# Ajax0564/VyomAI

Hardware: AMD Instinct MI355X
Metric: training tokens/sec (12L d=768 seq=512 GPT-style decoder, CLM) (higher is better)
Workload: dtype bf16; 1 GPU; configs[1]: GPT-style Decoder 12L d=768 h=12 RoPE vocab 50265, CLM training B=32/GPU seq=512, AdamW, bf16 kernels + fp32 masters; global_batch=32, seq_len=512, parallelism=dp1, attention=none, weights=deterministic recipe (vyomai_amd.recipe)

## Files before the change

include/vyom_hip.h:

```cpp
#ifndef VYOM_HIP_H
#define VYOM_HIP_H

#include <stdint.h>

#ifdef __cplusplus
extern "C" {
#endif

typedef enum { VY_F32 = 0, VY_BF16 = 1 } vy_dtype;

typedef enum {
  VY_OK = 0,
  VY_ERR_ARG = -1,
  VY_ERR_UNSUPPORTED = -2,
  VY_ERR_LAUNCH = -3
} vy_status;

typedef enum {
  VY_ACT_NONE = 0, VY_ACT_GELU_ERF = 1, VY_ACT_GELU_TANH = 2,
  VY_ACT_SILU = 3, VY_ACT_TANH = 4, VY_ACT_SIGMOID = 5, VY_ACT_RELU6 = 6, VY_ACT_LEAKY_RELU = 7
} vy_act;
#define VY_ACT_SAVE_DERIV 0x100

enum {
// ... 42 lines not shown
                        void* v_cache, int64_t max_blocks, int block_size, int64_t T, int h, int hk, int dh,
                        int dtype, void* stream);
int vy_paged_qknorm_rope_write(void* qkv, int64_t ld, const int32_t* positions, const int64_t* slot_mapping,
                               const float* cos_tab, const float* sin_tab, int64_t table_rows,
                               const float* q_scale, const float* k_scale, float eps, void* k_cache,
                               void* v_cache, int64_t max_blocks, int block_size, int64_t T, int h, int hk, int dh,
                               int dtype, void* stream);
int vy_attn_paged_decode(const void* q, int64_t q_ld, const int32_t* q_rows, const void* k_cache,
                         const void* v_cache, int64_t max_blocks, int block_size,
                         const int32_t* block_table, int64_t bt_stride, const int32_t* seqlens,
                         int64_t max_seqlen, void* out, int64_t o_ld, int64_t B, int h, int hk, int dh,
                         float scale, int n_split, void* ws, int64_t ws_bytes, int dtype, void* stream);
int64_t vy_attn_paged_decode_ws_bytes(int64_t B, int h, int hk, int dh, int64_t max_seqlen, int n_split, int dtype);
int vy_attn_paged_prefill(const void* q, int64_t q_ld, const void* k_cache, const void* v_cache,
                          int64_t max_blocks, int block_size, const int32_t* block_table, int64_t bt_stride,
                          const int32_t* cu_q, const int32_t* ctx_lens, int64_t n_seq, int64_t max_q,
                          int64_t max_kv, void* out, int64_t o_ld, int h, int hk, int dh, float scale,
                          int dtype, void* stream);
int vy_paged_gather(const void* k_cache, const void* v_cache, int64_t max_blocks, int block_size,
                    const int32_t* block_table, int64_t n_blocks, int64_t S, void* k_out, void* v_out,
                    int hk, int dh, int dtype, void* stream);

int vy_layernorm_fwd(const void* x, int64_t ldx, const void* gamma, const void* beta, void* y,
                     int64_t ldy, float* mean, float* rstd, int64_t M, int64_t N, float eps,
                     int dtype, void* stream);

int vy_rmsnorm_fwd(const void* x, int64_t ldx, const void* w, void* y, int64_t ldy, int64_t M,
                   int64_t N, float eps, float w_offset, int dtype, void* stream);

int vy_gated_act_fwd(const void* gate_up, int64_t ldg, void* out, int64_t ldo, int64_t M, int64_t I,
                     int act, int dtype, void* stream);

int vy_rmsnorm_bwd(const void* dy, int64_t lddy, const void* x, int64_t ldx, const void* w,
                   const void* add_to, int64_t ldadd, void* dx, int64_t lddx, float* dw, float beta,
                   float* ws, int64_t M, int64_t N, float eps, float w_offset, int dtype, void* stream);

int vy_gated_act_bwd(const void* d_act, int64_t lddo, const void* gate_up, int64_t ldg, void* d_gate_up,
                     int64_t lddg, int64_t M, int64_t I, int act, int dtype, void* stream);

int vy_rope_fwd(void* x, int64_t sb, int64_t sh, int64_t sl, const float* cos_tab,
                const float* sin_tab, int64_t pos0, int64_t B, int heads, int64_t L, int dh,
                int inverse, int dtype, void* stream);


int vy_linear_dgrad(const void* dy, int64_t lddy, const void* wt, int64_t ldwt, const void* pre,
                    int64_t ldpre, int act, const void* add_to, int64_t ldadd, const void* add_to2,
                    int64_t ldadd2, void* dx, int64_t lddx, int64_t M, int64_t N, int64_t K, int dtype,
                    void* stream);

int vy_linear_wgrad(const void* dy, int64_t lddy, const void* x, int64_t ldx, float* dw,
                    int64_t lddw, float* db, float beta, const float* alpha_dev, int64_t M, int64_t N,
                    int64_t K, int dtype, void* stream);

typedef struct vy_wgrad_desc {
  const void* dy; int64_t lddy;
  const void* x; int64_t ldx;
  float* dw; int64_t lddw;
  float* db;
  int64_t M, N, K;
} vy_wgrad_desc;
int vy_linear_wgrad_grouped(const vy_wgrad_desc* descs, int32_t n, int dtype, void* stream);

typedef struct vy_colsum_desc {
  float* ws; int32_t W, N;
  float* out0; float* out1;
  int32_t acc;
} vy_colsum_desc;
int vy_linear_wgrad_grouped_cs(const vy_wgrad_desc* descs, int32_t n, const vy_colsum_desc* cs, int32_t ncs, int dtype,
                               void* stream);

int64_t vy_layernorm_bwd_ws_rows(int64_t M);
int vy_layernorm_bwd(const void* dy, int64_t lddy, const void* x, int64_t ldx, const void* gamma,
                     const float* mean, const float* rstd, void* dx, int64_t lddx, float* dgamma,
                     float* dbeta, float beta, float* ws, int64_t M, int64_t N, int dtype,
                     void* stream);
int vy_layernorm_bwd_partial(const void* dy, int64_t lddy, const void* x, int64_t ldx, const void* gamma,
                             const float* mean, const float* rstd, void* dx, int64_t lddx, float* ws, int64_t M,
                             int64_t N, int dtype, void* stream);

int vy_attn_bwd(const void* q, int64_t q_sb, int64_t q_sh, int64_t q_sl,
                const void* k, int64_t k_sb, int64_t k_sh, int64_t k_sl,
                const void* v, int64_t v_sb, int64_t v_sh, int64_t v_sl,
                const void* out, const void* dout, int64_t o_sb, int64_t o_sl, const float* lse,
                float* delta_ws,
                void* dq, int64_t dq_sb, int64_t dq_sh, int64_t dq_sl,
                void* dk, int64_t dk_sb, int64_t dk_sh, int64_t dk_sl,
                void* dv, int64_t dv_sb, int64_t dv_sh, int64_t dv_sl,
                int mask_kind, int64_t start_pos, const uint8_t* keypad, int64_t kp_sb,
                const float* cos_tab, const float* sin_tab, int64_t rope_pos0,
                int64_t B, int h, int hk, int64_t L, int64_t S, int dh, float scale, int dtype,
                void* stream);

int vy_ddp_unique_id(void* id128);
int vy_ddp_init(const void* id128, int rank, int world);
int vy_ddp_world(void);
int vy_ddp_rank(void);
int vy_ddp_all_reduce_async(void* buf, int64_t count, int dtype, void* stream);
int vy_ddp_destroy(void);

int vy_adamw_step(float* p, const float* g, float* m, float* v, void* p_bf16, int64_t n, float lr,
                  float beta1, float beta2, float eps, float weight_decay, int64_t step,
                  float grad_scale, const float* grad_scale_dev, void* stream);
int vy_adamw_step_gated(float* p, const float* g, float* m, float* v, void* p_bf16, int64_t n, float lr,
                        float beta1, float beta2, float eps, float weight_decay, int64_t step,
                        float grad_scale, const float* grad_scale_dev, const float* gate, void* stream);

// ... 119 lines not shown
```

vyomai_amd/_lib.py:

```python
from __future__ import annotations

import ctypes as C
import os
from typing import Optional

_HERE = os.path.dirname(os.path.abspath(__file__))
LIB_PATH = os.environ.get("VY_LIB_PATH") or os.path.join(_HERE, "lib", "libvyom_hip.so")

VY_F32, VY_BF16 = 0, 1
ACT_NONE, ACT_GELU_ERF, ACT_GELU_TANH = 0, 1, 2
ACT_SILU, ACT_TANH, ACT_SIGMOID, ACT_RELU6, ACT_LEAKY_RELU = 3, 4, 5, 6, 7
ACT_SAVE_DERIV = 0x100
MASK_NONE, MASK_CAUSAL, MASK_KEYPAD, MASK_ADDITIVE = 0, 1, 2, 4

_p, _i64, _i, _f, _u64 = C.c_void_p, C.c_int64, C.c_int, C.c_float, C.c_uint64

PROTOTYPES = {
    "vy_linear_fwd": [_p, _i64, _p, _i64, _p, _p, _i64, _p, _i64, _p, _i64, _i64, _i64, _i, _i, _p],
    "vy_qkv_rope_fwd": [_p, _i64, _p, _i64, _p, _p, _p, _i64,
                        _p, _i64, _i64, _i64, _p, _i64, _i64, _i64, _p, _i64, _i64, _i64,
                        _i64, _i64, _i64, _i, _i, _i, _i, _p],
    "vy_attn_fwd": [_p, _i64, _i64, _i64, _p, _i64, _i64, _i64, _p, _i64, _i64, _i64,
                    _p, _i64, _i64, _p, _i, _i64, _p, _i64, _p, _i64, _i64,
                    _i64, _i, _i, _i64, _i64, _i, _f, _i, _p],
# ... 6 lines not shown
                             _p, _i64, _i, _p],
    "vy_attn_paged_prefill": [_p, _i64, _p, _p, _i64, _i, _p, _i64, _p, _p, _i64, _i64, _i64, _p, _i64, _i, _i, _i, _f,
                              _i, _p],
    "vy_paged_gather": [_p, _p, _i64, _i, _p, _i64, _i64, _p, _p, _i, _i, _i, _p],
    "vy_layernorm_fwd": [_p, _i64, _p, _p, _p, _i64, _p, _p, _i64, _i64, _f, _i, _p],
    "vy_rmsnorm_fwd": [_p, _i64, _p, _p, _i64, _i64, _i64, _f, _f, _i, _p],
    "vy_gated_act_fwd": [_p, _i64, _p, _i64, _i64, _i64, _i, _i, _p],
    "vy_rmsnorm_bwd": [_p, _i64, _p, _i64, _p, _p, _i64, _p, _i64, _p, _f, _p, _i64, _i64, _f, _f, _i, _p],
    "vy_gated_act_bwd": [_p, _i64, _p, _i64, _p, _i64, _i64, _i64, _i, _i, _p],
    "vy_rope_fwd": [_p, _i64, _i64, _i64, _p, _p, _i64, _i64, _i, _i64, _i, _i, _i, _p],
    "vy_linear_dgrad": [_p, _i64, _p, _i64, _p, _i64, _i, _p, _i64, _p, _i64, _p, _i64, _i64, _i64, _i64, _i, _p],
    "vy_linear_wgrad": [_p, _i64, _p, _i64, _p, _i64, _p, _f, _p, _i64, _i64, _i64, _i, _p],
    "vy_linear_wgrad_grouped": [_p, _i, _i, _p],
    "vy_linear_wgrad_grouped_cs": [_p, _i, _p, _i, _i, _p],
    "vy_layernorm_bwd_partial": [_p, _i64, _p, _i64, _p, _p, _p, _p, _i64, _p, _i64, _i64, _i, _p],
    "vy_layernorm_bwd": [_p, _i64, _p, _i64, _p, _p, _p, _p, _i64, _p, _p, _f, _p, _i64, _i64, _i, _p],
    "vy_attn_bwd": [_p, _i64, _i64, _i64, _p, _i64, _i64, _i64, _p, _i64, _i64, _i64,
                    _p, _p, _i64, _i64, _p, _p,
                    _p, _i64, _i64, _i64, _p, _i64, _i64, _i64, _p, _i64, _i64, _i64,
                    _i, _i64, _p, _i64, _p, _p, _i64, _i64, _i, _i, _i64, _i64, _i, _f, _i, _p],
    "vy_adamw_step": [_p, _p, _p, _p, _p, _i64, _f, _f, _f, _f, _f, _i64, _f, _p, _p],
    "vy_adamw_step_gated": [_p, _p, _p, _p, _p, _i64, _f, _f, _f, _f, _f, _i64, _f, _p, _p, _p],
    "vy_sumsq": [_p, _i64, _p, _p, _p],
    "vy_linear_dropout_fwd": [_p, _i64, _p, _i64, _p, _p, _i64, _p, _i64, _i64, _i64, _i64, _f, _u64, _u64, _i, _p],
    "vy_dropout": [_p, _i64, _p, _i64, _i64, _i64, _f, _u64, _u64, _i, _p],
    "vy_act_bwd": [_p, _i64, _p, _i64, _p, _i64, _i64, _i64, _i, _i, _p],
    "vy_xent_fwd": [_p, _i64, _p, _i64, _p, _p, _p, _i64, _i64, _p, _i, _p],
    "vy_xent_bwd": [_p, _i64, _p, _i64, _p, _p, _p, _i64, _i64, _i, _p],
    "vy_xent_fused": [_p, _i64, _p, _i64, _p, _p, _p, _p, _i64, _i64, _p, _i, _p],
    "vy_xent_sample_fwd": [_p, _i64, _p, _i64, _p, _p, _p, _p, _f, _u64, _u64, _i64, _i64, _p, _i, _p],
    "vy_xent_sample_fused": [_p, _i64, _p, _i64, _p, _p, _p, _p, _p, _f, _u64, _u64, _i64, _i64, _p, _i, _p],
    "vy_gumbel_noise": [_p, _i64, _i64, _i64, _u64, _u64, _p],
    "vy_bce_head_fwd": [_p, _i64, _p, _p, _p, _p, _p, _p, _i64, _i64, _i, _p],
    "vy_bce_head_bwd": [_p, _i64, _p, _p, _p, _p, _p, _p, _p, _i64, _p, _p, _i, _i64, _i64, _i, _p],
    "vy_mlm_mask": [_p, _i64, _p, _i, _f, _i64, _i64, _i64, _u64, _u64, _p, _p, _p, _p],
    "vy_logprob_fwd": [_p, _i64, _p, _p, _p, _p, _i64, _i64, _p, _i, _p],
    "vy_logprob_bwd": [_p, _i64, _p, _p, _p, _i64, _i64, _i, _p],
    "vy_logprob_fused": [_p, _i64, _p, _p, _p, _p, _i64, _i64, _p, _i, _p],
    "vy_transpose_batched": [_p, _i, _i, _i, _p],
    "vy_embedding_fwd": [_p, _i64, _p, _p, _i64, _i64, _i64, _i64, _p, _i, _p],
    "vy_embedding_bwd": [_p, _i64, _p, _p, _i64, _i64, _i64, _i64, _i64, _i, _p],
    "vy_transpose": [_p, _i64, _p, _i64, _i64, _i64, _i, _p],
    "vy_greedy_step": [_p, _i64, _i64, _i64, _i, _p, _i64, _i64, _p, _i64, _p, _i, _p, _p, _p],
    "vy_sampling_probs": [_p, _i64, _i64, _i64, _i, _f, _i, _f, _p, _i64, _p],
    "vy_decoder_step": [_p, _p, _i64, _p, _p, _p, _i64, _p],
    "vy_gemma_decoder_step": [_p, _p, _i64, _p, _i64, _p],
    "vy_cast": [_p, _p, _i64, _i, _i, _p],
    "vy_ddp_unique_id": [_p],
    "vy_ddp_init": [_p, _i, _i],
    "vy_ddp_all_reduce_async": [_p, _i64, _i, _p],
    "vy_ddp_destroy": [],
    "vy_set_concurrent_chains": [_i],
    "vy_workspace_set": [_p, _p, _i64],
}
OTHER_SYMBOLS = ["vy_last_error", "vy_abi_version", "vy_layernorm_bwd_ws_rows", "vy_decode_ws_bytes",
                 "vy_gemma_ws_bytes", "vy_ddp_world", "vy_ddp_rank", "vy_attn_paged_decode_ws_bytes"]
ALL_SYMBOLS = list(PROTOTYPES) + OTHER_SYMBOLS


class VyWgradDesc(C.Structure):
    _fields_ = [("dy", _p), ("lddy", _i64), ("x", _p), ("ldx", _i64), ("dw", _p), ("lddw", _i64), ("db", _p),
                ("M", _i64), ("N", _i64), ("K", _i64)]


class VyColsumDesc(C.Structure):
    _fields_ = [("ws", _p), ("W", C.c_int32), ("N", C.c_int32), ("out0", _p), ("out1", _p), ("acc", C.c_int32)]


class VyomHipError(RuntimeError):
    pass


_lib: Optional[C.CDLL] = None


def load() -> C.CDLL:
    global _lib
    if _lib is not None:
        return _lib
    if not os.path.exists(LIB_PATH):
        raise VyomHipError(
            f"{LIB_PATH} is missing: build it with `python -c 'import __graft_entry__ as g; g.build()'` "
            "(hipcc --offload-arch=gfx950).  vyomai_amd has no CPU or PyTorch fallback."
        )
    lib = C.CDLL(LIB_PATH)
    for name, argtypes in PROTOTYPES.items():
        fn = getattr(lib, name)
        fn.argtypes = argtypes
        fn.restype = C.c_int
    lib.vy_last_error.restype = C.c_char_p
    lib.vy_last_error.argtypes = []
    lib.vy_abi_version.restype = C.c_int
    lib.vy_layernorm_bwd_ws_rows.restype = C.c_int64
    lib.vy_layernorm_bwd_ws_rows.argtypes = [_i64]
    lib.vy_decode_ws_bytes.restype = C.c_int64
    lib.vy_decode_ws_bytes.argtypes = [C.c_int32] * 7
    lib.vy_attn_paged_decode_ws_bytes.restype = C.c_int64
    lib.vy_attn_paged_decode_ws_bytes.argtypes = [_i64, _i, _i, _i, _i64, _i, _i]
    _lib = lib
    return lib


def call(name: str, *args) -> None:
    lib = load()
    rc = getattr(lib, name)(*args)
    if rc != 0:
        raise VyomHipError(f"{name} failed ({rc}): {lib.vy_last_error().decode()}")


def dtype_code(torch_dtype) -> int:
    import torch

    if torch_dtype == torch.bfloat16:
        return VY_BF16
    if torch_dtype == torch.float32:
        return VY_F32
    raise VyomHipError(f"vyomai_amd kernels support float32 and bfloat16, got {torch_dtype}")
```

vyomai_amd/csrc/vy_bwd.hip:

```cpp
#include "vy_attn_tile.h"
#include <float.h>
#include <stdlib.h>
#include <string.h>

namespace {


__device__ __forceinline__ int xcd_remap(int bid, int nwg) {
  const int xcd = bid & 7, q = nwg >> 3, r = nwg & 7;
  return (xcd < r ? xcd * (q + 1) : r * (q + 1) + (xcd - r) * q) + (bid >> 3);
}

__device__ __forceinline__ bf16x8 tr_pair(const char* base, int row_bytes) {
  const s16x4 lo = __builtin_amdgcn_ds_read_tr16_b64_v4i16((VY_LDS s16x4*)(base));
  const s16x4 hi = __builtin_amdgcn_ds_read_tr16_b64_v4i16((VY_LDS s16x4*)(base + 8 * row_bytes));
  union { struct { s16x4 a, b; } s; bf16x8 v; } u;
  u.s.a = lo; u.s.b = hi;
  return u.v;
}

typedef __attribute__((ext_vector_type(2))) __bf16 bf16x2_t;

template <int BT, int MS_, bool MF16>
struct WgradTile {
// ... 17 lines not shown
    wave = wave_, m_begin = m_begin_, m_end = m_end_;
    nst = (m_end - m_begin + MS - 1) / MS;
    ragged = ((m_end - m_begin) % MS) != 0;
    zero = reinterpret_cast<const bf16*>(vy_zero16);
    sources(dY, lddy, n0, N, lane, a_ptr, a_step);
    sources(X, ldx, k0, K, lane, b_ptr, b_step);
  }
  __device__ __forceinline__ void sources(const bf16* __restrict__ src, int64_t ld, int c0, int C, int lane,
                                          const bf16* (&ptr)[PP], int64_t (&step)[PP]) {
#pragma unroll
    for (int t = 0; t < PP; ++t) {
      const int P = (wave * PP + t) * 1024 + lane * 16;
      const int r = P / ROWB, off = P % ROWB;
      const int col = (off ^ (((r & 3) << 6) | (MF16 ? ((r >> 2) & 1) << 5 : 0))) >> 1;
      const bool ok = c0 + col < C;
      row[t] = r;
      ptr[t] = ok ? src + (int64_t)(m_begin + r) * ld + c0 + col : zero;
      step[t] = ok ? (int64_t)MS * ld : 0;
    }
  }
  __device__ __forceinline__ void issue(const bf16* (&ptr)[PP], const int64_t (&step)[PP], int s, char* dst) {
    const bool tail = ragged && s == nst - 1;
    const int rows = m_end - (m_begin + s * MS);
#pragma unroll
    for (int t = 0; t < PP; ++t) {
      const bf16* p = (tail && row[t] >= rows) ? zero : ptr[t];
      __builtin_amdgcn_global_load_lds((const VY_GLOBAL void*)p, (VY_LDS void*)(dst + (wave * PP + t) * 1024), 16, 0, 0);
      ptr[t] += step[t];
    }
  }
  __device__ __forceinline__ void stage(int s, char* dst) {
    issue(a_ptr, a_step, s, dst);
    issue(b_ptr, b_step, s, dst + TILE);
  }
};

__device__ __forceinline__ float wgrad_db_dot(const bf16x8& a, float s) {
  const bf16x2_t ones2 = {(__bf16)1.0f, (__bf16)1.0f};
  union { bf16x8 v; bf16x2_t h[4]; } u_;
  u_.v = a;
#pragma unroll
  for (int e = 0; e < 4; ++e) s = __builtin_amdgcn_fdot2_f32_bf16(u_.h[e], ones2, s, false);
  return s;
}

template <class T>
struct WgradMma32 {
  static constexpr int TJ = T::WKT / 32, KS = T::MS / 16, ROWB = T::ROWB;
  f32x16 acc[2][TJ];
  float sdb[2];
  int fr, fh;
  unsigned a_lds[2], b_lds[TJ];

  __device__ __forceinline__ WgradMma32(const char* smem, int lane, int wn, int wk) {
#pragma unroll
    for (int i = 0; i < 2; ++i)
#pragma unroll
      for (int j = 0; j < TJ; ++j)
#pragma unroll
        for (int r = 0; r < 16; ++r) acc[i][j][r] = 0.f;
    sdb[0] = sdb[1] = 0.f;
    fr = lane & 31, fh = lane >> 5;
    const int li = lane & 15, g16 = (lane >> 4) & 1;
    const int tr_row = 4 * fh + (li >> 2);
    const int tr_sw = ((li >> 2) & 3) << 6;
    const int a_rd = (2 * (wn * 64 + 16 * g16 + 4 * (li & 3)));
    const int b_rd = (2 * (wk * T::WKT + 16 * g16 + 4 * (li & 3)));
#pragma unroll
    for (int i = 0; i < 2; ++i) a_lds[i] = vy_lds_addr(smem) + tr_row * ROWB + ((a_rd + 64 * i) ^ tr_sw);
#pragma unroll
    for (int j = 0; j < TJ; ++j) b_lds[j] = vy_lds_addr(smem) + tr_row * ROWB + ((b_rd + 64 * j) ^ tr_sw);
  }
  __device__ __forceinline__ void mma_stage(unsigned off, bool do_db) {
    unsigned a_base[2], b_base[TJ];
#pragma unroll
    for (int i = 0; i < 2; ++i) a_base[i] = a_lds[i] + off;
#pragma unroll
    for (int j = 0; j < TJ; ++j) b_base[j] = b_lds[j] + off;
    bf16x8 af[2][2], bfr[2][TJ];
    auto frags = [&](auto ks_c, bf16x8* a_, bf16x8* b_) {
      constexpr int ks = decltype(ks_c)::value;
#pragma unroll
      for (int i = 0; i < 2; ++i)
        a_[i] = vy_lds_tr16_pair_off<16 * ks * ROWB, (16 * ks + 8) * ROWB>(a_base[i]);
#pragma unroll
      for (int j = 0; j < TJ; ++j)
        b_[j] = vy_lds_tr16_pair_off<T::TILE + 16 * ks * ROWB, T::TILE + (16 * ks + 8) * ROWB>(b_base[j]);
    };
    frags(std::integral_constant<int, 0>{}, af[0], bfr[0]);
    vy_static_for<KS>([&](auto ks_c) {
      constexpr int ks = decltype(ks_c)::value;
      constexpr int c_ = ks & 1;
      if constexpr (ks < KS - 1) {
        frags(std::integral_constant<int, ks + 1>{}, af[c_ ^ 1], bfr[c_ ^ 1]);
        asm volatile("s_waitcnt lgkmcnt(%0)" ::"n"(2 * (2 + TJ)) : "memory");
      } else {
        asm volatile("s_waitcnt lgkmcnt(0)" ::: "memory");
      }
#pragma unroll
      for (int i = 0; i < 2; ++i) vy_tie(af[c_][i]);
#pragma unroll
      for (int j = 0; j < TJ; ++j) vy_tie(bfr[c_][j]);
#pragma unroll
      for (int i = 0; i < 2; ++i)
#pragma unroll
        for (int j = 0; j < TJ; ++j)
          acc[i][j] = __builtin_amdgcn_mfma_f32_32x32x16_bf16(af[c_][i], bfr[c_][j], acc[i][j], 0, 0, 0);
      if (do_db) {
#pragma unroll
        for (int i = 0; i < 2; ++i) sdb[i] = wgrad_db_dot(af[c_][i], sdb[i]);
      }
    });
  }
  __device__ __forceinline__ void epilogue(float* __restrict__ dW, int64_t lddw, float* __restrict__ db, bool do_db,
                                           float alpha, int nw, int kw, int N, int K) {
    if (do_db) {
#pragma unroll
      for (int i = 0; i < 2; ++i) {
        const float t_ = (sdb[i] + __shfl_xor(sdb[i], 32, 64)) * alpha;
        const int n = nw + 32 * i + fr;
        if (fh == 0 && n < N) atomicAdd(db + n, t_);
      }
    }
#pragma unroll
    for (int i = 0; i < 2; ++i)
#pragma unroll
      for (int j = 0; j < TJ; ++j) {
        const int k = kw + 32 * j + fr;
        if (k >= K) continue;
#pragma unroll
        for (int r = 0; r < 16; ++r) {
          const int n = nw + 32 * i + (r & 3) + 8 * (r >> 2) + 4 * fh;
          if (n < N) atomicAdd(dW + (int64_t)n * lddw + k, acc[i][j][r] * alpha);
        }
      }
  }
};

template <class T>
struct WgradMma16 {
  static constexpr int TI = 4, TJ = T::WKT / 16, KS = T::MS / 32, JH = TJ / 2, ROWB = T::ROWB;
  f32x4 acc[TI][TJ];
  float sdb[TI];
  int r16, kq;
  unsigned a_lds[TI], b_lds[TJ];

  __device__ __forceinline__ WgradMma16(const char* smem, int lane, int wn, int wk) {
#pragma unroll
    for (int i = 0; i < TI; ++i)
#pragma unroll
      for (int j = 0; j < TJ; ++j) acc[i][j] = f32x4{0.f, 0.f, 0.f, 0.f};
#pragma unroll
    for (int i = 0; i < TI; ++i) sdb[i] = 0.f;
    r16 = lane & 15, kq = lane >> 4;
    const int q_ = r16 >> 2, p_ = r16 & 3;
    const int sw16 = (q_ << 6) | ((kq & 1) << 5);
#pragma unroll
    for (int i = 0; i < TI; ++i) a_lds[i] = vy_lds_addr(smem) + (4 * kq + q_) * ROWB + ((2 * (wn * 64 + 16 * i + 4 * p_)) ^ sw16);
#pragma unroll
    for (int j = 0; j < TJ; ++j)
      b_lds[j] = vy_lds_addr(smem) + (4 * kq + q_) * ROWB + ((2 * (wk * T::WKT + 16 * j + 4 * p_)) ^ sw16);
  }
  __device__ __forceinline__ void mma_stage(unsigned off, bool do_db) {
    unsigned a_base[TI], b_base[TJ];
#pragma unroll
    for (int i = 0; i < TI; ++i) a_base[i] = a_lds[i] + off;
#pragma unroll
    for (int j = 0; j < TJ; ++j) b_base[j] = b_lds[j] + off;
    vy_static_for<KS>([&](auto ks_c) {
      constexpr int ks = decltype(ks_c)::value;
      bf16x8 af[TI], bfr[TJ];
      vy_static_for<TI>([&](auto i_c) {
        constexpr int i = decltype(i_c)::value;
        af[i] = vy_lds_tr16_pair_off<32 * ks * ROWB, (32 * ks + 16) * ROWB>(a_base[i]);
      });
      vy_static_for<TJ>([&](auto j_c) {
        constexpr int j = decltype(j_c)::value;
        bfr[j] = vy_lds_tr16_pair_off<T::TILE + 32 * ks * ROWB, T::TILE + (32 * ks + 16) * ROWB>(b_base[j]);
      });
      asm volatile("s_waitcnt lgkmcnt(%0)" ::"n"(2 * JH) : "memory");
#pragma unroll
      for (int i = 0; i < TI; ++i) vy_tie(af[i]);
#pragma unroll
      for (int j = 0; j < JH; ++j) vy_tie(bfr[j]);
#pragma unroll
      for (int i = 0; i < TI; ++i)
#pragma unroll
        for (int j = 0; j < JH; ++j)
          acc[i][j] = __builtin_amdgcn_mfma_f32_16x16x32_bf16(af[i], bfr[j], acc[i][j], 0, 0, 0);
      asm volatile("s_waitcnt lgkmcnt(0)" ::: "memory");
#pragma unroll
      for (int j = JH; j < TJ; ++j) vy_tie(bfr[j]);
#pragma unroll
      for (int i = 0; i < TI; ++i)
#pragma unroll
        for (int j = JH; j < TJ; ++j)
          acc[i][j] = __builtin_amdgcn_mfma_f32_16x16x32_bf16(af[i], bfr[j], acc[i][j], 0, 0, 0);
      if (do_db) {
#pragma unroll
        for (int i = 0; i < TI; ++i) sdb[i] = wgrad_db_dot(af[i], sdb[i]);
      }
    });
  }
  __device__ __forceinline__ void epilogue(float* __restrict__ dW, int64_t lddw, float* __restrict__ db, bool do_db,
                                           float alpha, int nw, int kw, int N, int K) {
    if (do_db) {
#pragma unroll
      for (int i = 0; i < TI; ++i) {
        float t_ = sdb[i];
        t_ += __shfl_xor(t_, 16, 64);
        t_ += __shfl_xor(t_, 32, 64);
        const int n = nw + 16 * i + r16;
        if (kq == 0 && n < N) atomicAdd(db + n, t_ * alpha);
      }
    }
    const bool hi = kq >= 2;
#pragma unroll
    for (int i = 0; i < TI; ++i)
#pragma unroll
      for (int jp = 0; jp < JH; ++jp) {
        const int k = kw + 16 * (2 * jp + (hi ? 1 : 0)) + r16;
#pragma unroll
        for (int r = 0; r < 4; ++r) {
          const unsigned x = __builtin_bit_cast(unsigned, acc[i][2 * jp][r] * alpha);
          const unsigned y = __builtin_bit_cast(unsigned, acc[i][2 * jp + 1][r] * alpha);
          auto sw = __builtin_amdgcn_permlane32_swap(x, y, false, false);
          const int nlo = nw + 16 * i + 4 * (kq & 1) + r;
          if (k < K) {
            if (nlo < N) atomicAdd(dW + (int64_t)nlo * lddw + k, __builtin_bit_cast(float, (unsigned)sw[0]));
            if (nlo + 8 < N) atomicAdd(dW + (int64_t)(nlo + 8) * lddw + k, __builtin_bit_cast(float, (unsigned)sw[1]));
          }
        }
      }
  }
};

template <int BN, int BKW, int MS, int NS, bool MF16>
__device__ __forceinline__ void wgrad_tn_bf16_body(
    const bf16* __restrict__ dY, int64_t lddy, const bf16* __restrict__ X, int64_t ldx,
    float* __restrict__ dW, int64_t lddw, float* __restrict__ db, const float* __restrict__ alpha_dev,
    int M, int N, int K, int tiles_k, int tiles_nk, int m_chunk, int diag, int wg) {
  static_assert(BN == BKW && ((BN == 128 && MS == 64 && NS == 2) || (BN == 256 && MS == 32 && NS == 4)),
                "built shapes: 128 x 128 x 64 in 2 stages, 256 x 256 x 32 in 4");
  typedef WgradTile<BN, MS, MF16> Tile;
  typedef std::conditional_t<MF16, WgradMma16<Tile>, WgradMma32<Tile>> Mma;
  constexpr int STAGE = Tile::STAGE, PS = 2 * Tile::PP;
  __shared__ __attribute__((aligned(16))) char smem[NS * STAGE];
  const int tid = threadIdx.x, lane = tid & 63;
  const int wave = __builtin_amdgcn_readfirstlane(tid >> 6);
  const int wn = wave >> 1, wk = wave & 1;
  const int split = wg / tiles_nk, t2 = wg - split * tiles_nk;
  const int tile_n = t2 / tiles_k, tile_k = t2 - tile_n * tiles_k;
  const int n0 = tile_n * BN, k0 = tile_k * BKW;
  const int m_begin = split * m_chunk;
  const int m_end = min(M, m_begin + m_chunk);
  if (m_begin >= m_end) return;

  Tile t(dY, lddy, X, ldx, n0, k0, N, K, m_begin, m_end, wave, lane);
  const bool do_db = db != nullptr && tile_k == 0 && wk == 0;
  Mma mma(smem, lane, wn, wk);
  const int nst = t.nst;
#pragma unroll
  for (int s_ = 0; s_ < NS - 1; ++s_)
    if (s_ < nst) t.stage(s_, smem + s_ * STAGE);
  for (int s = 0; s < nst; ++s) {
    const int younger = min(NS - 2, nst - 1 - s);
    if (younger >= 2) asm volatile("s_waitcnt vmcnt(%0)" ::"n"(2 * PS) : "memory");
    else if (younger == 1) asm volatile("s_waitcnt vmcnt(%0)" ::"n"(PS) : "memory");
    else asm volatile("s_waitcnt vmcnt(0)" ::: "memory");
    __builtin_amdgcn_s_barrier();
    asm volatile("" ::: "memory");
    if (s + NS - 1 < nst) t.stage(s + NS - 1, smem + (s + NS - 1) % NS * STAGE);
    mma.mma_stage(s % NS * STAGE, do_db);
  }
  if (diag == 1) {
    if (mma.acc[0][0][0] == 12345.678f) dW[0] = 1.f;
    return;
  }
  const float alpha = alpha_dev ? *alpha_dev : 1.0f;
  mma.epilogue(dW, lddw, db, do_db, alpha, n0 + wn * 64, k0 + wk * Tile::WKT, N, K);
}

template <int BN, int BKW, int MS, int NS, bool MF16>
__global__ __launch_bounds__(BN * 2, BN == 128 ? 2 : 1) void wgrad_tn_bf16_kernel(
    const bf16* __restrict__ dY, int64_t lddy, const bf16* __restrict__ X, int64_t ldx,
    float* __restrict__ dW, int64_t lddw, float* __restrict__ db, const float* __restrict__ alpha_dev,
    int M, int N, int K, int tiles_k, int tiles_nk, int m_chunk, int diag) {
  wgrad_tn_bf16_body<BN, BKW, MS, NS, MF16>(dY, lddy, X, ldx, dW, lddw, db, alpha_dev, M, N, K, tiles_k, tiles_nk, m_chunk,
                                            diag, xcd_remap(blockIdx.x, gridDim.x));
}

struct WgradItem {
  const bf16* dY; const bf16* X; float* dW; float* db;
  int64_t lddy, ldx, lddw;
  int M, N, K, tiles_k, tiles_nk, m_chunk, item0;
};
struct WgradGroup { WgradItem g[8]; int n; };

struct ColsumItem { const float* ws; float* out0; float* out1; int W, N, rps, acc, blk0; };
struct ColsumGroup { ColsumItem c[8]; int n; int items; };

__device__ __forceinline__ void colsum_slab_block(const ColsumItem& it, int blk) {
  __shared__ float red[2][2][4][64];
  const int tid = threadIdx.x;
  const int c = tid & 63, g = (tid >> 6) & 3, h = tid >> 8;
  const int n = blk * 64 + c;
  const int W = it.W, N = it.N, rps = it.rps;
  const float* __restrict__ ws = it.ws;
  const bool one = rps >= W;
  float ta = 0.f, tb = 0.f;
  for (int s0 = 0; s0 * rps < W; s0 += 2) {
    const int w0 = (s0 + h) * rps, w1 = min(W, w0 + rps);
    float a = 0.f, b = 0.f;
    if (n < N) {
      for (int wb = w0 + g; wb < w1; wb += 32) {
        float av[8], bv[8];
#pragma unroll
        for (int i = 0; i < 8; ++i) {
          const int w = wb + 4 * i;
          const int wc = w < w1 ? w : wb;
          av[i] = ws[(int64_t)wc * N + n];
          bv[i] = ws[(int64_t)(W + wc) * N + n];
        }
#pragma unroll
        for (int i = 0; i < 8; ++i)
          if (wb + 4 * i < w1) { a += av[i]; b += bv[i]; }
      }
    }
    red[h][0][g][c] = a; red[h][1][g][c] = b;
    __syncthreads();
    if (tid < 64) {
#pragma unroll
      for (int hh = 0; hh < 2; ++hh)
        if ((s0 + hh) * rps < W) {
          const float sa = red[hh][0][0][c] + red[hh][0][1][c] + red[hh][0][2][c] + red[hh][0][3][c];
          const float sb = red[hh][1][0][c] + red[hh][1][1][c] + red[hh][1][2][c] + red[hh][1][3][c];
          ta = one ? sa : ta + sa;
          tb = one ? sb : tb + sb;
        }
    }
    __syncthreads();
  }
// ... 388 lines not shown
    const int n = n0 + 4 * ty + i;
    if (n >= N) continue;
#pragma unroll
    for (int j = 0; j < 4; ++j) {
      const int k = k0 + 4 * tx + j;
      if (k < K) atomicAdd(dW + (int64_t)n * lddw + k, alpha * acc[i][j]);
    }
  }
  if (db && k0 == 0) {
    sb[lr][lc] = colsum;
    __syncthreads();
    if (tid < 64 && n0 + tid < N) atomicAdd(db + n0 + tid, alpha * (sb[0][tid] + sb[1][tid] + sb[2][tid] + sb[3][tid]));
  }
}

int wgrad_f32(const char* who, const void* dy, int64_t lddy, const void* x, int64_t ldx, float* dw, int64_t lddw, float* db,
              float beta, const float* alpha_dev, int64_t M, int64_t N, int64_t K, hipStream_t st) {
  if (beta == 0.f) {
    if (hipMemset2DAsync(dw, lddw * sizeof(float), 0, K * sizeof(float), N, st) != hipSuccess)
      VY_FAIL(VY_ERR_LAUNCH, "%s: memset failed", who);
    if (db && hipMemsetAsync(db, 0, N * sizeof(float), st) != hipSuccess) VY_FAIL(VY_ERR_LAUNCH, "%s: memset failed", who);
  }
  const int tiles_k = (int)vy_cdiv(K, 64), tiles = (int)vy_cdiv(N, 64) * tiles_k;
  int64_t splits = vy_cdiv(1024, tiles);
  const int64_t max_splits = vy_cdiv(M, 64);
  if (splits > max_splits) splits = max_splits;
  if (splits < 1) splits = 1;
  const int64_t m_chunk = vy_cdiv(vy_cdiv(M, splits), 16) * 16;
  splits = vy_cdiv(M, m_chunk);
  hipLaunchKernelGGL(wgrad_tn_f32_kernel, dim3((unsigned)(tiles * splits)), dim3(256), 0, st, (const float*)dy, lddy,
                     (const float*)x, ldx, dw, lddw, db, alpha_dev, (int)M, (int)N, (int)K, tiles_k, tiles, (int)m_chunk);
  VY_CHECK_LAUNCH(who);
  return VY_OK;
}

bool wgrad_bf16_operands_ok(const void* dy, int64_t lddy, const void* x, int64_t ldx, int64_t N, int64_t K) {
  return !(K % 8 || lddy % 8 || ldx % 8 || lddy < vy_cdiv(N, 8) * 8 || (uintptr_t)dy % 16 || (uintptr_t)x % 16);
}

struct WgradSplit { int64_t splits, m_chunk; };
WgradSplit wgrad_split(int64_t M, int64_t want) {
  const int64_t max_splits = vy_cdiv(M, 256);
  if (want > max_splits) want = max_splits;
  if (want < 1) want = 1;
  const int64_t m_chunk = vy_cdiv(vy_cdiv(M, want), 64) * 64;
  return {vy_cdiv(M, m_chunk), m_chunk};
}

int wgrad_env(const char* name, int dflt) { const char* e = getenv(name); return e ? atoi(e) : dflt; }

int wgrad_m16() { static const int v = wgrad_env("VY_WGRAD_M16", 1); return v; }
int wgrad_diag() { static const int v = wgrad_env("VY_WGRAD_DIAG", 0); return v; }

}

extern "C" int vy_linear_wgrad(const void* dy, int64_t lddy, const void* x, int64_t ldx, float* dw,
                               int64_t lddw, float* db, float beta, const float* alpha_dev, int64_t M,
                               int64_t N, int64_t K, int dtype, void* stream) {
  const char* who = "vy_linear_wgrad";
  if (dtype != VY_BF16 && dtype != VY_F32) VY_FAIL(VY_ERR_ARG, "%s: bad dtype %d", who, dtype);
  if (!dy || !x || !dw || M <= 0 || N <= 0 || K <= 0) VY_FAIL(VY_ERR_ARG, "%s: bad arguments", who);
  if (dtype == VY_F32) {
    if (beta != 0.f && beta != 1.f) VY_FAIL(VY_ERR_ARG, "%s: beta must be 0 or 1", who);
    return wgrad_f32(who, dy, lddy, x, ldx, dw, lddw, db, beta, alpha_dev, M, N, K, (hipStream_t)stream);
  }
  if (!wgrad_bf16_operands_ok(dy, lddy, x, ldx, N, K))
    VY_FAIL(VY_ERR_ARG, "%s: K and leading dimensions must be multiples of 8 (lddy >= roundup8(N)), operands 16-byte aligned", who);
  if (beta != 0.f && beta != 1.f) VY_FAIL(VY_ERR_ARG, "%s: beta must be 0 or 1", who);
  static const int wv = wgrad_env("VY_WGRAD_VARIANT", -1);
  static const int tgt = wgrad_env("VY_WGRAD_TARGET", 0);
  if (wv != -1 && wv != 0 && wv != 8)
    VY_FAIL(VY_ERR_UNSUPPORTED, "%s: VY_WGRAD_VARIANT=%d was removed (the values left are 0 and 8; unset selects by shape)", who, wv);
  hipStream_t st = (hipStream_t)stream;
  if (beta == 0.f) {
    if (hipMemset2DAsync(dw, lddw * sizeof(float), 0, K * sizeof(float), N, st) != hipSuccess)
      VY_FAIL(VY_ERR_LAUNCH, "%s: memset failed", who);
    if (db && hipMemsetAsync(db, 0, N * sizeof(float), st) != hipSuccess)
      VY_FAIL(VY_ERR_LAUNCH, "%s: memset failed", who);
  }
  const bool big = wv < 0 ? (N >= 8192 && M >= 4096) : wv == 8;
  const int BT = big ? 256 : 128;
  const int tiles_k = (int)vy_cdiv(K, BT), tiles = (int)vy_cdiv(N, BT) * tiles_k;
  const WgradSplit sp = wgrad_split(M, tgt > 0 ? vy_cdiv(tgt, tiles) : big ? 256 / tiles : vy_cdiv(384, tiles));
  const int w16 = wgrad_m16();
  auto kernel = big ? (w16 ? wgrad_tn_bf16_kernel<256, 256, 32, 4, true> : wgrad_tn_bf16_kernel<256, 256, 32, 4, false>)
                    : (w16 >= 2 ? wgrad_tn_bf16_kernel<128, 128, 64, 2, true> : wgrad_tn_bf16_kernel<128, 128, 64, 2, false>);
  hipLaunchKernelGGL(kernel, dim3((unsigned)(tiles * sp.splits)), dim3(BT * 2), 0, st, (const bf16*)dy, lddy, (const bf16*)x,
                     ldx, dw, lddw, db, alpha_dev, (int)M, (int)N, (int)K, tiles_k, tiles, (int)sp.m_chunk, wgrad_diag());
  VY_CHECK_LAUNCH(who);
  return VY_OK;
}

static int wgrad_grouped(const char* who, const vy_wgrad_desc* descs, int32_t n, const vy_colsum_desc* cs, int32_t ncs,
                        int dtype, void* stream) {
  if (dtype != VY_BF16 && dtype != VY_F32) VY_FAIL(VY_ERR_ARG, "%s: bad dtype %d", who, dtype);
  if (n < 0 || n > 8 || (n > 0 && !descs) || ncs < 0 || ncs > 8 || (ncs > 0 && !cs) || n + ncs == 0)
    VY_FAIL(VY_ERR_ARG, "%s: 1..8 descriptors", who);
  for (int i = 0; i < ncs; ++i)
    if (!cs[i].ws || cs[i].W <= 0 || cs[i].N <= 0 || (cs[i].acc != 0 && cs[i].acc != 1))
      VY_FAIL(VY_ERR_ARG, "%s: column-sum descriptor %d: bad arguments", who, i);
  if (dtype == VY_F32) {
    for (int i = 0; i < ncs; ++i)
      if (int rc = vy_ln_colsum(cs[i].ws, cs[i].W, cs[i].N, cs[i].out0, cs[i].out1, cs[i].acc, (hipStream_t)stream)) return rc;
    for (int i = 0; i < n; ++i) {
      const vy_wgrad_desc& d = descs[i];
      if (!d.dy || !d.x || !d.dw || d.M <= 0 || d.N <= 0 || d.K <= 0) VY_FAIL(VY_ERR_ARG, "%s: descriptor %d: bad arguments", who, i);
      if (int rc = wgrad_f32(who, d.dy, d.lddy, d.x, d.ldx, d.dw, d.lddw, d.db, 1.f, nullptr, d.M, d.N, d.K, (hipStream_t)stream)) return rc;
    }
    return VY_OK;
  }
  int64_t tiles_total = 0;
  for (int i = 0; i < n; ++i) {
    const vy_wgrad_desc& d = descs[i];
    if (!d.dy || !d.x || !d.dw || d.M <= 0 || d.N <= 0 || d.K <= 0) VY_FAIL(VY_ERR_ARG, "%s: descriptor %d: bad arguments", who, i);
    if (!wgrad_bf16_operands_ok(d.dy, d.lddy, d.x, d.ldx, d.N, d.K))
      VY_FAIL(VY_ERR_ARG, "%s: descriptor %d: K and leading dimensions must be multiples of 8, operands 16-byte aligned", who, i);
    tiles_total += vy_cdiv(d.N, 256) * vy_cdiv(d.K, 256);
  }
  static const int tgt = wgrad_env("VY_WGRAD_GROUP_TARGET", 256);
  WgradGroup grp;
  memset(&grp, 0, sizeof(grp));
  grp.n = n;
  int64_t items = 0;
  for (int i = 0; i < n; ++i) {
    const vy_wgrad_desc& d = descs[i];
    const int64_t tiles_k = vy_cdiv(d.K, 256), tiles = vy_cdiv(d.N, 256) * tiles_k;
    const WgradSplit sp = wgrad_split(d.M, tgt / tiles_total);
    WgradItem& it = grp.g[i];
    it.dY = (const bf16*)d.dy; it.X = (const bf16*)d.x; it.dW = d.dw; it.db = d.db;
    it.lddy = d.lddy; it.ldx = d.ldx; it.lddw = d.lddw;
    it.M = (int)d.M; it.N = (int)d.N; it.K = (int)d.K;
    it.tiles_k = (int)tiles_k; it.tiles_nk = (int)tiles; it.m_chunk = (int)sp.m_chunk; it.item0 = (int)items;
    items += tiles * sp.splits;
  }
  for (int i = n; i < 8; ++i) grp.g[i] = grp.g[0];
  ColsumGroup cg;
  memset(&cg, 0, sizeof(cg));
// ... 554 lines not shown
```

Measured before the change: 872,800 tokens/s.

## Add persistent load-balanced ranged wgrad kernel for large-N weight gradients

Adds a persistent wgrad kernel for the 256x256 tile path, launched with one workgroup per CU. Each workgroup walks a contiguous range of (N-tile, M-block) segments for a fixed K-tile and runs the staged MMA ring on each segment. It writes each segment's partial result through the existing epilogue, then zeroes its accumulators and continues. This targets the tail imbalance of the old fixed grid of tiles×splits blocks on large-vocabulary shapes such as the LM head. The cost is more epilogue writes when one workgroup spans several N-tiles or splits a tile, plus new debug hooks for overriding and inspecting the plan.

Result: no change. 881,500 tokens/s (median of 6 runs) (+1.0%).

```diff
diff --git a/include/vyom_hip.h b/include/vyom_hip.h
--- a/include/vyom_hip.h
+++ b/include/vyom_hip.h
@@ -118,6 +118,9 @@
                     int64_t lddw, float* db, float beta, const float* alpha_dev, int64_t M, int64_t N,
                     int64_t K, int dtype, void* stream);
 
+int vy_debug_set_wgrad_balance(int on, int slots);
+int vy_debug_wgrad_plan(int64_t M, int64_t N, int64_t K, int slots, int target, int wg, int32_t* out, int cap);
+
 typedef struct vy_wgrad_desc {
   const void* dy; int64_t lddy;
   const void* x; int64_t ldx;
diff --git a/vyomai_amd/_lib.py b/vyomai_amd/_lib.py
--- a/vyomai_amd/_lib.py
+++ b/vyomai_amd/_lib.py
@@ -82,9 +82,11 @@
     "vy_ddp_destroy": [],
     "vy_set_concurrent_chains": [_i],
     "vy_workspace_set": [_p, _p, _i64],
+    "vy_debug_set_wgrad_balance": [_i, _i],
 }
 OTHER_SYMBOLS = ["vy_last_error", "vy_abi_version", "vy_layernorm_bwd_ws_rows", "vy_decode_ws_bytes",
-                 "vy_gemma_ws_bytes", "vy_ddp_world", "vy_ddp_rank", "vy_attn_paged_decode_ws_bytes"]
+                 "vy_gemma_ws_bytes", "vy_ddp_world", "vy_ddp_rank", "vy_attn_paged_decode_ws_bytes",
+                 "vy_debug_wgrad_plan"]
 ALL_SYMBOLS = list(PROTOTYPES) + OTHER_SYMBOLS
 
 
@@ -127,6 +129,8 @@
     lib.vy_decode_ws_bytes.argtypes = [C.c_int32] * 7
     lib.vy_attn_paged_decode_ws_bytes.restype = C.c_int64
     lib.vy_attn_paged_decode_ws_bytes.argtypes = [_i64, _i, _i, _i, _i64, _i, _i]
+    lib.vy_debug_wgrad_plan.restype = C.c_int
+    lib.vy_debug_wgrad_plan.argtypes = [_i64, _i64, _i64, _i, _i, _i, C.POINTER(C.c_int32), _i]
     _lib = lib
     return lib
 
diff --git a/vyomai_amd/csrc/vy_bwd.hip b/vyomai_amd/csrc/vy_bwd.hip
--- a/vyomai_amd/csrc/vy_bwd.hip
+++ b/vyomai_amd/csrc/vy_bwd.hip
@@ -93,7 +93,7 @@
   int fr, fh;
   unsigned a_lds[2], b_lds[TJ];
 
-  __device__ __forceinline__ WgradMma32(const char* smem, int lane, int wn, int wk) {
+  __device__ __forceinline__ void zero() {
 #pragma unroll
     for (int i = 0; i < 2; ++i)
 #pragma unroll
@@ -101,6 +101,9 @@
 #pragma unroll
         for (int r = 0; r < 16; ++r) acc[i][j][r] = 0.f;
     sdb[0] = sdb[1] = 0.f;
+  }
+  __device__ __forceinline__ WgradMma32(const char* smem, int lane, int wn, int wk) {
+    zero();
     fr = lane & 31, fh = lane >> 5;
     const int li = lane & 15, g16 = (lane >> 4) & 1;
     const int tr_row = 4 * fh + (li >> 2);
@@ -186,13 +189,16 @@
   int r16, kq;
   unsigned a_lds[TI], b_lds[TJ];
 
+  __device__ __forceinline__ void zero() {
+#pragma unroll
+    for (int i = 0; i < TI; ++i)
+#pragma unroll
+      for (int j = 0; j < TJ; ++j) acc[i][j] = f32x4{0.f, 0.f, 0.f, 0.f};
+#pragma unroll
+    for (int i = 0; i < TI; ++i) sdb[i] = 0.f;
+  }
   __device__ __forceinline__ WgradMma16(const char* smem, int lane, int wn, int wk) {
-#pragma unroll
-    for (int i = 0; i < TI; ++i)
-#pragma unroll
-      for (int j = 0; j < TJ; ++j) acc[i][j] = f32x4{0.f, 0.f, 0.f, 0.f};
-#pragma unroll
-    for (int i = 0; i < TI; ++i) sdb[i] = 0.f;
+    zero();
     r16 = lane & 15, kq = lane >> 4;
     const int q_ = r16 >> 2, p_ = r16 & 3;
     const int sw16 = (q_ << 6) | ((kq & 1) << 5);
@@ -276,30 +282,9 @@
   }
 };
 
-template <int BN, int BKW, int MS, int NS, bool MF16>
-__device__ __forceinline__ void wgrad_tn_bf16_body(
-    const bf16* __restrict__ dY, int64_t lddy, const bf16* __restrict__ X, int64_t ldx,
-    float* __restrict__ dW, int64_t lddw, float* __restrict__ db, const float* __restrict__ alpha_dev,
-    int M, int N, int K, int tiles_k, int tiles_nk, int m_chunk, int diag, int wg) {
-  static_assert(BN == BKW && ((BN == 128 && MS == 64 && NS == 2) || (BN == 256 && MS == 32 && NS == 4)),
-                "built shapes: 128 x 128 x 64 in 2 stages, 256 x 256 x 32 in 4");
-  typedef WgradTile<BN, MS, MF16> Tile;
-  typedef std::conditional_t<MF16, WgradMma16<Tile>, WgradMma32<Tile>> Mma;
+template <int NS, class Tile, class Mma>
+__device__ __forceinline__ void wgrad_ring(Tile& t, Mma& mma, char* smem, bool do_db) {
   constexpr int STAGE = Tile::STAGE, PS = 2 * Tile::PP;
-  __shared__ __attribute__((aligned(16))) char smem[NS * STAGE];
-  const int tid = threadIdx.x, lane = tid & 63;
-  const int wave = __builtin_amdgcn_readfirstlane(tid >> 6);
-  const int wn = wave >> 1, wk = wave & 1;
-  const int split = wg / tiles_nk, t2 = wg - split * tiles_nk;
-  const int tile_n = t2 / tiles_k, tile_k = t2 - tile_n * tiles_k;
-  const int n0 = tile_n * BN, k0 = tile_k * BKW;
-  const int m_begin = split * m_chunk;
-  const int m_end = min(M, m_begin + m_chunk);
-  if (m_begin >= m_end) return;
-
-  Tile t(dY, lddy, X, ldx, n0, k0, N, K, m_begin, m_end, wave, lane);
-  const bool do_db = db != nullptr && tile_k == 0 && wk == 0;
-  Mma mma(smem, lane, wn, wk);
   const int nst = t.nst;
 #pragma unroll
   for (int s_ = 0; s_ < NS - 1; ++s_)
@@ -314,6 +299,32 @@
     if (s + NS - 1 < nst) t.stage(s + NS - 1, smem + (s + NS - 1) % NS * STAGE);
     mma.mma_stage(s % NS * STAGE, do_db);
   }
+}
+
+template <int BN, int BKW, int MS, int NS, bool MF16>
+__device__ __forceinline__ void wgrad_tn_bf16_body(
+    const bf16* __restrict__ dY, int64_t lddy, const bf16* __restrict__ X, int64_t ldx,
+    float* __restrict__ dW, int64_t lddw, float* __restrict__ db, const float* __restrict__ alpha_dev,
+    int M, int N, int K, int tiles_k, int tiles_nk, int m_chunk, int diag, int wg) {
+  static_assert(BN == BKW && ((BN == 128 && MS == 64 && NS == 2) || (BN == 256 && MS == 32 && NS == 4)),
+                "built shapes: 128 x 128 x 64 in 2 stages, 256 x 256 x 32 in 4");
+  typedef WgradTile<BN, MS, MF16> Tile;
+  typedef std::conditional_t<MF16, WgradMma16<Tile>, WgradMma32<Tile>> Mma;
+  __shared__ __attribute__((aligned(16))) char smem[NS * Tile::STAGE];
+  const int tid = threadIdx.x, lane = tid & 63;
+  const int wave = __builtin_amdgcn_readfirstlane(tid >> 6);
+  const int wn = wave >> 1, wk = wave & 1;
+  const int split = wg / tiles_nk, t2 = wg - split * tiles_nk;
+  const int tile_n = t2 / tiles_k, tile_k = t2 - tile_n * tiles_k;
+  const int n0 = tile_n * BN, k0 = tile_k * BKW;
+  const int m_begin = split * m_chunk;
+  const int m_end = min(M, m_begin + m_chunk);
+  if (m_begin >= m_end) return;
+
+  Tile t(dY, lddy, X, ldx, n0, k0, N, K, m_begin, m_end, wave, lane);
+  const bool do_db = db != nullptr && tile_k == 0 && wk == 0;
+  Mma mma(smem, lane, wn, wk);
+  wgrad_ring<NS>(t, mma, smem, do_db);
   if (diag == 1) {
     if (mma.acc[0][0][0] == 12345.678f) dW[0] = 1.f;
     return;
@@ -329,6 +340,81 @@
     int M, int N, int K, int tiles_k, int tiles_nk, int m_chunk, int diag) {
   wgrad_tn_bf16_body<BN, BKW, MS, NS, MF16>(dY, lddy, X, ldx, dW, lddw, db, alpha_dev, M, N, K, tiles_k, tiles_nk, m_chunk,
                                             diag, xcd_remap(blockIdx.x, gridDim.x));
+}
+
+struct WgradPlan { int tiles_k, nblk, groups, R, total; };
+
+__host__ bool wgrad_plan_make(int64_t M, int64_t N, int64_t K, int64_t slots, int64_t items, WgradPlan* p) {
+  const int64_t tiles_k = vy_cdiv(K, 256), tiles_n = vy_cdiv(N, 256), nblk = vy_cdiv(M, 64);
+  if (slots < tiles_k || items <= slots) return false;
+  const int64_t groups = slots / tiles_k, total = tiles_n * nblk, R = vy_cdiv(total, groups);
+  if (R < nblk || total > INT32_MAX) return false;
+  *p = WgradPlan{(int)tiles_k, (int)nblk, (int)groups, (int)R, (int)total};
+  return true;
+}
+
+struct WgradWalk { int cur, end, tail_b, tail_e; };
+
+__host__ __device__ __forceinline__ bool wgrad_plan_range(const WgradPlan& p, int id, int* tile_k, WgradWalk* w) {
+  const int g = id / p.tiles_k;
+  *tile_k = id - g * p.tiles_k;
+  const int b = g * p.R;
+  const int e = p.total - b < p.R ? p.total : b + p.R;
+  if (g >= p.groups || b >= e) return false;
+  const int r = b % p.nblk;
+  const int bt = r == 0 ? b : (e - b < p.nblk - r ? e : b + (p.nblk - r));
+  if (bt < e) *w = WgradWalk{bt, e, b, bt};
+  else *w = WgradWalk{b, e, 0, 0};
+  return true;
+}
+__host__ __device__ __forceinline__ int wgrad_plan_segment(const WgradPlan& p, const WgradWalk& w, int* mb, int* me) {
+  const int tile_n = w.cur / p.nblk;
+  *mb = w.cur - tile_n * p.nblk;
+  *me = w.end - w.cur < p.nblk - *mb ? *mb + (w.end - w.cur) : p.nblk;
+  return tile_n;
+}
+__host__ __device__ __forceinline__ bool wgrad_plan_advance(WgradWalk* w, int done) {
+  w->cur += done;
+  if (w->cur < w->end) return true;
+  if (w->tail_b >= w->tail_e) return false;
+  w->cur = w->tail_b, w->end = w->tail_e, w->tail_b = w->tail_e;
+  return true;
+}
+
+template <int BN, int BKW, int MS, int NS, bool MF16>
+__global__ __launch_bounds__(BN * 2, 1) void wgrad_tn_bf16_ranged_kernel(
+    const bf16* __restrict__ dY, int64_t lddy, const bf16* __restrict__ X, int64_t ldx,
+    float* __restrict__ dW, int64_t lddw, float* __restrict__ db, const float* __restrict__ alpha_dev,
+    int M, int N, int K, WgradPlan plan, int diag) {
+  static_assert(BN == 256 && BKW == 256 && MS == 32 && NS == 4, "the 256 x 256 tile only");
+  typedef WgradTile<BN, MS, MF16> Tile;
+  typedef std::conditional_t<MF16, WgradMma16<Tile>, WgradMma32<Tile>> Mma;
+  __shared__ __attribute__((aligned(16))) char smem[NS * Tile::STAGE];
+  const int tid = threadIdx.x, lane = tid & 63;
+  const int wave = __builtin_amdgcn_readfirstlane(tid >> 6);
+  const int wn = wave >> 1, wk = wave & 1;
+  int tile_k;
+  WgradWalk walk;
+  if (!wgrad_plan_range(plan, xcd_remap(blockIdx.x, gridDim.x), &tile_k, &walk)) return;
+  const int k0 = tile_k * BKW;
+  const bool do_db = db != nullptr && tile_k == 0 && wk == 0;
+  Mma mma(smem, lane, wn, wk);
+  while (true) {
+    int mb, me;
+    const int n0 = wgrad_plan_segment(plan, walk, &mb, &me) * BN;
+    Tile t(dY, lddy, X, ldx, n0, k0, N, K, mb * 64, min(M, me * 64), wave, lane);
+    wgrad_ring<NS>(t, mma, smem, do_db);
+    if (diag == 1) {
+      if (mma.acc[0][0][0] == 12345.678f) dW[0] = 1.f;
+    } else {
+      const float alpha = alpha_dev ? *alpha_dev : 1.0f;
+      mma.epilogue(dW, lddw, db, do_db, alpha, n0 + wn * 64, k0 + wk * Tile::WKT, N, K);
+    }
+    if (!wgrad_plan_advance(&walk, me - mb)) break;
+    __builtin_amdgcn_s_barrier();
+    asm volatile("" ::: "memory");
+    mma.zero();
+  }
 }
 
 struct WgradItem {
@@ -823,6 +909,45 @@
 int wgrad_m16() { static const int v = wgrad_env("VY_WGRAD_M16", 1); return v; }
 int wgrad_diag() { static const int v = wgrad_env("VY_WGRAD_DIAG", 0); return v; }
 
+int g_wgrad_balance = -1, g_wgrad_slots = 0;
+int wgrad_balance() {
+  if (g_wgrad_balance < 0) g_wgrad_balance = wgrad_env("VY_WGRAD_BALANCE", 1) ? 1 : 0;
+  return g_wgrad_balance;
+}
+int wgrad_slots() {
+  if (g_wgrad_slots > 0) return g_wgrad_slots;
+  static const int cus = [] {
+    int dev = 0, n = 0;
+    if (hipGetDevice(&dev) != hipSuccess || hipDeviceGetAttribute(&n, hipDeviceAttributeMultiprocessorCount, dev) != hipSuccess)
+      n = 0;
+    return n;
+  }();
+  return cus;
+}
+
+}
+
+extern "C" int vy_debug_set_wgrad_balance(int on, int slots) {
+  g_wgrad_balance = on ? 1 : 0;
+  g_wgrad_slots = slots > 0 ? slots : 0;
+  return 0;
+}
+
+extern "C" int vy_debug_wgrad_plan(int64_t M, int64_t N, int64_t K, int slots, int target, int wg, int32_t* out, int cap) {
+  if (M <= 0 || N <= 0 || K <= 0 || slots <= 0 || target <= 0 || wg < 0 || wg >= slots || cap < 0 || (cap > 0 && !out))
+    return -2;
+  const int64_t tiles = vy_cdiv(N, 256) * vy_cdiv(K, 256);
+  WgradPlan p;
+  if (!wgrad_plan_make(M, N, K, slots, tiles * wgrad_split(M, target / tiles).splits, &p)) return -1;
+  int tile_k, n = 0, mb, me;
+  WgradWalk w;
+  if (!wgrad_plan_range(p, wg, &tile_k, &w)) return 0;
+  do {
+    const int tile_n = wgrad_plan_segment(p, w, &mb, &me);
+    if (n < cap) { out[4 * n] = tile_n; out[4 * n + 1] = tile_k; out[4 * n + 2] = mb; out[4 * n + 3] = me; }
+    ++n;
+  } while (wgrad_plan_advance(&w, me - mb));
+  return n;
 }
 
 extern "C" int vy_linear_wgrad(const void* dy, int64_t lddy, const void* x, int64_t ldx, float* dw,
@@ -849,11 +974,19 @@
     if (db && hipMemsetAsync(db, 0, N * sizeof(float), st) != hipSuccess)
       VY_FAIL(VY_ERR_LAUNCH, "%s: memset failed", who);
   }
-  const bool big = wv < 0 ? (N >= 8192 && M >= 4096) : wv == 8;
+  const bool big = g_wgrad_slots > 0 || (wv < 0 ? (N >= 8192 && M >= 4096) : wv == 8);
   const int BT = big ? 256 : 128;
   const int tiles_k = (int)vy_cdiv(K, BT), tiles = (int)vy_cdiv(N, BT) * tiles_k;
-  const WgradSplit sp = wgrad_split(M, tgt > 0 ? vy_cdiv(tgt, tiles) : big ? 256 / tiles : vy_cdiv(384, tiles));
+  const WgradSplit sp = wgrad_split(M, tgt > 0 ? vy_cdiv(tgt, tiles) : big ? (g_wgrad_slots > 0 ? g_wgrad_slots : 256) / tiles : vy_cdiv(384, tiles));
   const int w16 = wgrad_m16();
+  WgradPlan plan;
+  if (big && wgrad_balance() && M < INT32_MAX - 64 && wgrad_plan_make(M, N, K, wgrad_slots(), tiles * sp.splits, &plan)) {
+    auto ranged = w16 ? wgrad_tn_bf16_ranged_kernel<256, 256, 32, 4, true> : wgrad_tn_bf16_ranged_kernel<256, 256, 32, 4, false>;
+    hipLaunchKernelGGL(ranged, dim3((unsigned)wgrad_slots()), dim3(512), 0, st, (const bf16*)dy, lddy, (const bf16*)x, ldx, dw,
+                       lddw, db, alpha_dev, (int)M, (int)N, (int)K, plan, wgrad_diag());
+    VY_CHECK_LAUNCH(who);
+    return VY_OK;
+  }
   auto kernel = big ? (w16 ? wgrad_tn_bf16_kernel<256, 256, 32, 4, true> : wgrad_tn_bf16_kernel<256, 256, 32, 4, false>)
                     : (w16 >= 2 ? wgrad_tn_bf16_kernel<128, 128, 64, 2, true> : wgrad_tn_bf16_kernel<128, 128, 64, 2, false>);
   hipLaunchKernelGGL(kernel, dim3((unsigned)(tiles * sp.splits)), dim3(BT * 2), 0, st, (const bf16*)dy, lddy, (const bf16*)x,
```
